# HBioquant/DiffBindFR

Measured on AMD Instinct MI355X. Metric: poses_per_sec, higher is better.
Workload: dtype f32

## Files before the change

### diffbindfr_amd/csrc/api.cpp

```cpp
#include <cmath>
#include <cstdio>
#include <cstring>
#include <algorithm>
#include <atomic>
#include <map>

#include "common.h"

void launch_conv(const ConvArgs& a, hipStream_t st);
void launch_conv_layer(const ConvArgs* c4, hipStream_t st);
void launch_conv2(const Conv2Args& a, hipStream_t st);
void launch_conv2h(const Conv2Args& a, hipStream_t st);
void launch_convz(const ConvZArgs& a, hipStream_t st);
void launch_reduce_ln(const float* msg, const int* row_start, const int* row_cnt, int N, int D, const LNDesc& ln,
                      const float* old, int D_old, float* out, int ldo, int mode, hipStream_t st, const uint8_t* first = nullptr, unsigned long long sc_lanes = 0);
struct ReduceLayerArgs {
  const float* msg[4]; const int* row_start[4]; const int* row_cnt[4]; LNDesc ln[4];
  int NL, NA, D, D_old;
  const float* old_l; const float* old_a; float* out_l; float* out_a;
  const uint8_t* first[4]; unsigned long long sc_lanes[4];
};
static unsigned long long convz_sc_lanes(const ConvZ& z) {
  unsigned long long m = 0;
  for (int i = 0; i < z.n_io; ++i) m |= 0xfffull << (z.out_off[i] / 4);
// ... 7 lines not shown
  float lig_cut2, atom_cut2, cross_cut2;
  int lig_cap, atom_cap, dynamic_cross;
  EdgeSet set[N_SETS];
  int* err;
  int step, lds_nl, lds_na, n_chunk, lanes;
};
void dbfr_edge_form(const dbfr_batch& b, int* n_chunk, int* lanes);
void launch_edges(const GraphArgs& A, bool heads_only, hipStream_t st);
void launch_edge_log(const GraphArgs& A, int* log_row, int stride, hipStream_t st);
void launch_edge_ties(const GraphArgs& A, int* log_row, int stride, float tol, hipStream_t st);
void launch_graph_chunks(const GraphArgs& A, hipStream_t st);
void launch_flat_chunks(const int* tgt, const int* n_edges, int max_edges, int span, int n_span, int* cnt0, int cap, int* chunk_es, int* chunk_gl, hipStream_t st);
void launch_row_absmax(const float* lx, const int* lig_ptr, float* out_l, const float* ax, const int* atm_ptr, float* out_a, int ld, int D, int G, int n_rows_a, hipStream_t st);
void launch_batch_vectors(const dbfr_batch& b, int* lig_batch, int* atm_batch, uint8_t* is_cab, int* n_cab,
                          int* tor_batch, int* sc_batch, hipStream_t st);
void launch_time_embed(const float* t, int G, float emb_scale, float* temb, hipStream_t st);
enum MlpIn { IN_LIGNODE = 0, IN_LIGEDGE = 1, IN_TG = 2, IN_G = 3 };
struct MlpArgs {
  Mlp2 w; int mode; const int* n_rows_dev; int n_rows_max; const float* temb; const int* row_graph_tab; const int* tgt;
  const int* aux; const float* dist; const float* bond_feat; int nfeat; const float* lig_node; int nnode;
  const float* gs_offset; const float* gs_coeff; float* out;
};
void launch_mlp(const MlpArgs& a, hipStream_t st);
struct AtomEncArgs {
  const float* pocket_feat; const int* atm_batch; const float* temb; const float* emb[5]; int dims[5];
  const float* lin_t; int NA; float* out;
};
void launch_atom_encoder(const AtomEncArgs& a, hipStream_t st);
void launch_center_edges(const dbfr_batch& b, int* tgt, int* gth, float* dist, float* sh, int* row_start, int* row_cnt,
                         hipStream_t st);
struct TrRotArgs {
  const float* gp; const float* temb; const float* tr_sigma; const float* rot_norm; Mlp2 tr, rot; int G;
  int scale_by_sigma; float* tr_out; float* rot_out; int* err;
};
void launch_trrot(const TrRotArgs& a, hipStream_t st);
void launch_bond_attr(const float* x, int ldx, const int* b0, const int* b1, const int* bsel, int stride, int n,
                      float* out, hipStream_t st);
void launch_tor_final(const float* feat, const Mlp2& w, const float* norm2, int scale, int n, float* out, hipStream_t st);
struct SdeLigArgs {
  dbfr_batch b; const float* tr_score; const float* rot_score; const float* tor_score; const float* z_tr;
  const float* z_rot; const float* z_tor; float dt, tr_g2, tr_gsdt, rot_g2, rot_gsdt, tor_g2, tor_gsdt; float* traj;
  int* err;
};
void launch_sde_ligand(const SdeLigArgs& a, hipStream_t st);
void launch_sidechain(const dbfr_batch& b, const float* score, const float* z, float dt, float g2, float gsdt,
                      const int* a14_group, float* atom14_out, float* traj14, const int* err, hipStream_t st);
// ... 1072 lines not shown
  ga.lig_cut2 = cfg.lig_cutoff * cfg.lig_cutoff; ga.atom_cut2 = cfg.atom_cutoff * cfg.atom_cutoff;
  ga.cross_cut2 = cfg.dynamic_max_cross ? 1.0f : cfg.cross_cutoff * cfg.cross_cutoff;
  ga.lig_cap = cfg.lig_max_neighbors; ga.atom_cap = cfg.atom_max_neighbors; ga.dynamic_cross = cfg.dynamic_max_cross;
  for (int k = 0; k < N_SETS; ++k) ga.set[k] = w.set[k];
  ga.err = w.err; ga.step = step; ga.lds_nl = ga.lds_na = 0;
  dbfr_edge_form(*B, &ga.n_chunk, &ga.lanes);
  launch_edges(ga, false, st);
  if (int lrc = take_launch_error()) return lrc;
  if (m->gemm_split == DBFR_GEMM_REDUCE_FIRST) launch_graph_chunks(ga, st);
  if (m->edge_log && step < m->edge_log_steps) launch_edge_log(ga, m->edge_log + (size_t)step * N_SETS * m->edge_log_graphs, m->edge_log_graphs, st);
  if (m->tie_log && step < m->tie_log_steps) launch_edge_ties(ga, m->tie_log + (size_t)step * N_SETS * m->tie_log_graphs, m->tie_log_graphs, m->tie_tol, st);
  {
    MlpArgs a; memset(&a, 0, sizeof a);
    a.w = m->lig_node_emb; a.mode = IN_LIGNODE; a.n_rows_max = NL; a.temb = w.temb; a.row_graph_tab = w.lig_batch;
    a.lig_node = B->lig_node; a.nnode = cfg.lig_node_features; a.out = w.lig_x[0];
    launch_mlp(a, st);
  }
  {
    AtomEncArgs a; a.pocket_feat = B->pocket_feat; a.atm_batch = w.atm_batch; a.temb = w.temb;
    for (int i = 0; i < 5; ++i) { a.emb[i] = m->atom_emb[i]; a.dims[i] = m->atom_dims[i]; }
    a.lin_t = m->atom_lin_t; a.NA = NA; a.out = w.atom_x[0];
    launch_atom_encoder(a, st);
  }
  auto edge_mlp = [&](const Mlp2& mw, int mode, const EdgeSet& S, const int* tab, const float* off, const float* co) {
    MlpArgs a; memset(&a, 0, sizeof a);
    a.w = mw; a.mode = mode; a.n_rows_dev = S.n_edges; a.n_rows_max = S.cap; a.temb = w.temb; a.row_graph_tab = tab;
    a.tgt = S.tgt; a.aux = S.aux; a.dist = S.dist; a.bond_feat = B->bond_feat; a.nfeat = cfg.lig_edge_features;
    a.gs_offset = off; a.gs_coeff = co; a.out = S.emb;
    launch_mlp(a, st);
  };
  edge_mlp(m->lig_edge_emb, IN_LIGEDGE, w.set[SET_LL], w.lig_batch, m->gs_lig_off, m->gs_lig_c);
  edge_mlp(m->atom_edge_emb, IN_TG, w.set[SET_AA], w.atm_batch, m->gs_atom_off, m->gs_atom_c);
  edge_mlp(m->la_edge_emb, IN_TG, w.set[SET_AL], w.lig_batch, m->gs_cross_off, m->gs_cross_c);
  edge_mlp(m->la_edge_emb, IN_TG, w.set[SET_LA], w.atm_batch, m->gs_cross_off, m->gs_cross_c);
  static const int dims[4] = {48, 84, 120, 168};
  int cur = 0;
  for (int l = 0; l < cfg.num_conv_layers; ++l) {
    const int Di = dims[std::min(l, 3)], Do = dims[std::min(l + 1, 3)];
    const float *lx = w.lig_x[cur], *ax = w.atom_x[cur];
    float *lnew = w.lig_x[cur ^ 1], *anew = w.atom_x[cur ^ 1];
    const EdgeSet &LL = w.set[SET_LL], &AA = w.set[SET_AA], &AL = w.set[SET_AL], &LA = w.set[SET_LA];
    if (w.conv2 || l < m->conv2_layers) {
      const bool rf = m->gemm_split == DBFR_GEMM_REDUCE_FIRST && !((m->layer_fallback >> l) & 1u);
      const ConvW2* L2 = rf ? m->layer2v[l] : m->layer2[l];
      const Conv2Desc ds[4] = {
          conv2_desc(L2[0], LL.n_edges, LL.cap, LL.gth, LL.emb, LL.sh, lx, Di, LL.tgt, lx, Di, LL.gth, lx, Di, w.msg[0]),
          conv2_desc(L2[1], AL.n_edges, AL.cap, AL.gth, AL.emb, AL.sh, lx, Di, AL.tgt, ax, Di, AL.gth, ax, Di, w.msg[1]),
          conv2_desc(L2[2], AA.n_edges, AA.cap, AA.gth, AA.emb, AA.sh, ax, Di, AA.tgt, ax, Di, AA.gth, ax, Di, w.msg[2]),
          conv2_desc(L2[3], LA.n_edges, LA.cap, LA.gth, LA.emb, LA.sh, ax, Di, LA.tgt, lx, Di, LA.gth, lx, Di, w.msg[3])};
      const int Ws[4] = {m->layer[l][0].W, m->layer[l][1].W, m->layer[l][2].W, m->layer[l][3].W};
      if (rf) {
        launch_row_absmax(lx, B->lig_ptr, w.xmax_l, ax, B->atm_ptr, w.xmax_a, Di, Di, G, NA, st);
      }
      auto zd = [&](int i, const EdgeSet& S, const float* xmax) { return convz_desc(ds[i], m->layerz[l][i], S.tgt, Do, S.chunk_es, S.chunk_gl, S.chunk0 + G, S.chunk_cap, xmax); };
      const ConvZDesc zs[4] = {zd(0, LL, w.xmax_l), zd(1, AL, w.xmax_a), zd(2, AA, w.xmax_a), zd(3, LA, w.xmax_l)};
      conv2_call(m, ds, Ws, 4, st, (m->layer_fallback >> l) & 1u, rf ? zs : nullptr);
      ReduceLayerArgs ra;
// ... 481 lines not shown
extern "C" int dbfr_test_conv2(dbfr_model* m, int32_t layer, int32_t family, int32_t n_edges, const int32_t* n_edges_dev,
                               const int32_t* tgt, const int32_t* gth, const float* emb, const float* sh,
                               const float* tab1, int32_t ld1, const int32_t* idx1, const float* tab2, int32_t ld2,
                               const int32_t* idx2, const float* x, int32_t ldx, float* msg, void* hip_stream) {
  return test_conv_impl(m, true, layer, family, n_edges, n_edges_dev, tgt, gth, emb, sh, tab1, ld1, idx1, tab2, ld2, idx2, x, ldx,
                        msg, hip_stream);
}

extern "C" int dbfr_test_reduce_ln2(dbfr_model* m, int32_t layer, int32_t family, const float* msg, const int32_t* row_start, const int32_t* row_cnt,
                                    int32_t n_nodes, const float* old, int32_t d_old, float* out, int32_t mode, const uint8_t* seg_first, void* hip_stream) {
  if (!m) return fail(DBFR_ERR_ARG, "null model");
  const ConvW* cw = pick_conv(m, layer, family);
  if (!cw) return fail(DBFR_ERR_ARG, "no such conv");
  unsigned long long lanes = 0;
  if (seg_first) {
    if (layer == -1 || cw->K != 144) return fail(DBFR_ERR_ARG, "dbfr_test_reduce_ln2: seg_first with a conv that has no reduce-first form");
    lanes = convz_sc_lanes(layer >= 0 ? m->layerz[layer][family] : layer == -2 ? m->tor_convz : m->sc_convz);
  }
  launch_reduce_ln(msg, row_start, row_cnt, n_nodes, cw->D_out, cw->ln, old, d_old, out, cw->D_out, mode, (hipStream_t)hip_stream, seg_first, lanes);
  HIPCHECK(hipGetLastError());
  return DBFR_OK;
}

extern "C" int dbfr_test_reduce_ln(dbfr_model* m, int32_t layer, int32_t family, const float* msg,
                                   const int32_t* row_start, const int32_t* row_cnt, int32_t n_nodes, const float* old,
                                   int32_t d_old, float* out, int32_t mode, void* hip_stream) {
  if (!m) return fail(DBFR_ERR_ARG, "null model");
  const ConvW* cw = pick_conv(m, layer, family);
  if (!cw) return fail(DBFR_ERR_ARG, "no such conv");
  launch_reduce_ln(msg, row_start, row_cnt, n_nodes, cw->D_out, cw->ln, old, d_old, out, cw->D_out, mode,
                   (hipStream_t)hip_stream);
  HIPCHECK(hipGetLastError());
  return DBFR_OK;
}
```

### diffbindfr_amd/csrc/conv.hip

```cpp
#include <cstdio>
#include <cstdlib>
#include <type_traits>
#include <vector>

#include "common.h"

#ifndef CONV_PRIO
#define CONV_PRIO 0
#endif
#ifndef CONV_XPF
#define CONV_XPF 0
#endif
#ifndef CONV_NB2_WAVES
#define CONV_NB2_WAVES 2
#endif
#define XS_LD (MAXD + 4)

typedef float f32x4 __attribute__((ext_vector_type(4)));

#define TRACE_BLOCKS 1024
#define TRACE_TILES 48
#define TRACE_REC (2 + 3 * TRACE_TILES + 8)
#define RSTAMP(k) do { if ((ABL & 16) && a.trace && bid < TRACE_BLOCKS && lane == 0) a.trace[((size_t)bid * 4 + wave) * TRACE_REC + 2 + 3 * TRACE_TILES + (k)] = __builtin_amdgcn_s_memrealtime(); } while (0)
#define TSTAMP(k) do { if ((ABL & 16) && a.trace && bid < TRACE_BLOCKS && lane == 0) a.trace[((size_t)bid * 4 + wave) * TRACE_REC + 2 + 3 * TRACE_TILES + (k)] = __builtin_readcyclecounter(); } while (0)
// ... 500 lines not shown
      float v = buf[wave][c];
      float* o = out + (size_t)node * ldo + c;
      if (mode == 0) v = (c < D_old ? old[(size_t)node * D_old + c] : 0.f) + v;
      else if (mode == 1) v = *o + v;
      *o = v;
    }
  }
}

void launch_reduce_ln(const float* msg, const int* row_start, const int* row_cnt, int N, int D, const LNDesc& ln,
                      const float* old, int D_old, float* out, int ldo, int mode, hipStream_t st, const uint8_t* first, unsigned long long sc_lanes) {
  if (N <= 0) return;
  hipLaunchKernelGGL(k_reduce_ln, dim3((N + 3) / 4), dim3(256), 0, st, msg, row_start, row_cnt, N, D, ln, old, D_old,
                     out, ldo, mode, first, sc_lanes);
}

struct ReduceLayerArgs {
  const float* msg[4]; const int* row_start[4]; const int* row_cnt[4]; LNDesc ln[4];
  int NL, NA, D, D_old;
  const float* old_l; const float* old_a; float* out_l; float* out_a;
  const uint8_t* first[4]; unsigned long long sc_lanes[4];
};

__device__ __forceinline__ void mean_ln(const float* __restrict__ msg, int rs, int rc, int D, const LNDesc& ln, float* bw, int lane, const uint8_t* first, unsigned long long sc_lanes) {
  const int d4 = D >> 2;
  const f32x4 acc = row_sum(msg, rs, rc, D, lane, first, sc_lanes);
  if (lane < d4) {
    const float cntf = (float)max(rc, 1);
    bw[4 * lane] = acc[0] / cntf; bw[4 * lane + 1] = acc[1] / cntf; bw[4 * lane + 2] = acc[2] / cntf; bw[4 * lane + 3] = acc[3] / cntf;
  }
  __builtin_amdgcn_wave_barrier();
  int iw = 0, ib = 0;
  for (int bk = 0; bk < ln.nblk; ++bk) {
    const int mul = ln.mul[bk], dim = ln.dim[bk], off = ln.off[bk];
    const int nel = mul * dim;
    float mean[3] = {0.f, 0.f, 0.f};
    const bool d3 = dim == 3;
    for (int i = lane; i < nel; i += 64) {
      int comp = d3 ? i % 3 : 0;
      float v = bw[off + i];
      if (comp == 0) mean[0] += v; else if (comp == 1) mean[1] += v; else mean[2] += v;
    }
    for (int o = 32; o > 0; o >>= 1) mean[0] += __shfl_xor(mean[0], o);
    mean[0] /= (float)mul;
    if (d3) {
#pragma unroll
      for (int c = 1; c < 3; ++c) {
        for (int o = 32; o > 0; o >>= 1) mean[c] += __shfl_xor(mean[c], o);
        mean[c] /= (float)mul;
      }
    }
    float sq = 0.f;
    for (int i = lane; i < nel; i += 64) {
      int u = d3 ? i / 3 : i, comp = d3 ? i - 3 * u : 0;
      float v = bw[off + i] - (comp == 0 ? mean[0] : comp == 1 ? mean[1] : mean[2]) * ln.mean_shift[iw + u];
      bw[off + i] = v;
      sq += v * v;
    }
    __builtin_amdgcn_wave_barrier();
    for (int o = 32; o > 0; o >>= 1) sq += __shfl_xor(sq, o);
    const float inv = 1.0f / sqrtf(sq / (float)nel + 1e-5f);
    for (int i = lane; i < nel; i += 64) {
      int u = d3 ? i / 3 : i;
      float v = bw[off + i] * (inv * ln.weight[iw + u]);
      if (ln.is0e[bk]) v += ln.bias[ib + u];
      bw[off + i] = v;
    }
    iw += mul;
    if (ln.is0e[bk]) ib += mul;
  }
  __builtin_amdgcn_wave_barrier();
}

__global__ __launch_bounds__(256) void k_reduce_ln_layer(ReduceLayerArgs a) {
  __shared__ float buf[4][2][MAXD];
  const int lane = threadIdx.x & 63, wave = threadIdx.x >> 6;
  const int nbl = (a.NL + 3) / 4;
  const bool lig = (int)blockIdx.x < nbl;
  const int node = (lig ? blockIdx.x : blockIdx.x - nbl) * 4 + wave;
  const int N = lig ? a.NL : a.NA;
  if (node >= N) return;
  const int s0 = lig ? 0 : 2;
  mean_ln(a.msg[s0], a.row_start[s0][node], a.row_cnt[s0][node], a.D, a.ln[s0], buf[wave][0], lane, a.first[s0], a.sc_lanes[s0]);
  mean_ln(a.msg[s0 + 1], a.row_start[s0 + 1][node], a.row_cnt[s0 + 1][node], a.D, a.ln[s0 + 1], buf[wave][1], lane, a.first[s0 + 1], a.sc_lanes[s0 + 1]);
  const float* old = (lig ? a.old_l : a.old_a) + (size_t)node * a.D_old;
  float* out = (lig ? a.out_l : a.out_a) + (size_t)node * a.D;
#pragma unroll
  for (int j = 0; j < 3; ++j) {
    const int c = lane + 64 * j;
    if (c < a.D) out[c] = ((c < a.D_old ? old[c] : 0.f) + buf[wave][0][c]) + buf[wave][1][c];
  }
}

void launch_reduce_ln_layer(const ReduceLayerArgs& a, hipStream_t st) {
  const int nb = (a.NL + 3) / 4 + (a.NA + 3) / 4;
  if (nb <= 0) return;
  hipLaunchKernelGGL(k_reduce_ln_layer, dim3(nb), dim3(256), 0, st, a);
}
```

### diffbindfr_amd/csrc/graph.hip

```cpp
#include "common.h"

#define MAX_NL 256
#define MAX_NA 8192

enum SetKind { SET_LL = 0, SET_AA = 1, SET_AL = 2, SET_LA = 3, SET_TOR = 4, SET_SC = 5, N_SETS = 6 };

struct GraphArgs {
  dbfr_batch b;
  const int* lig_batch;
  const int* atm_batch;
  const uint8_t* is_cab;
  const int* n_cab;
  const float* tr_sigma;
  float lig_cut2, atom_cut2, cross_cut2;
  int lig_cap, atom_cap, dynamic_cross;
  EdgeSet set[N_SETS];
  int* err;
  int step;
  int lds_nl, lds_na;
  int n_chunk;
  int lanes;
};

__device__ __forceinline__ float d2_rn(float ax, float ay, float az, float bx, float by, float bz) {
// ... 747 lines not shown
#pragma unroll
  for (int t = 0; t < 3; ++t)
#pragma unroll
    for (int r = 0; r < 4; ++r) acc[t][r] = a.w.b1 ? a.w.b1[16 * t + 4 * g + r] : 0.f;
#pragma unroll
  for (int k = 0; k < NS; k += 4) {
    const float bv = hid[row][k + g];
#pragma unroll
    for (int t = 0; t < 3; ++t) acc[t] = __builtin_amdgcn_mfma_f32_16x16x4f32(w1[(k + g) * NS + 16 * t + n], bv, acc[t], 0, 0, 0);
  }
  if (row < nr) {
#pragma unroll
    for (int t = 0; t < 3; ++t) *reinterpret_cast<f32x4*>(a.out + (size_t)(r0 + row) * NS + 16 * t + 4 * g) = acc[t];
  }
  }
}

void launch_mlp(const MlpArgs& a, hipStream_t st) {
  if (a.n_rows_max <= 0) return;
  const int tiles = (a.n_rows_max + MLP_ROWS - 1) / MLP_ROWS;
  hipLaunchKernelGGL(k_mlp, dim3(tiles < 1024 ? tiles : 1024), dim3(256), 0, st, a);
}

struct AtomEncArgs {
  const float* pocket_feat;
  const int* atm_batch;
  const float* temb;
  const float* emb[5];
  int dims[5];
  const float* lin_t;
  int NA;
  float* out;
};

__global__ __launch_bounds__(256) void k_atom_encoder(AtomEncArgs a) {
  __shared__ float w[(NS + EMB) * NS];
  __shared__ float x[16][NS + EMB];
  for (int i = threadIdx.x; i < (NS + EMB) * NS; i += 256) w[i] = a.lin_t[i];
  const int r0 = blockIdx.x * 16;
  for (int i = threadIdx.x; i < 16 * (NS + EMB); i += 256) {
    int r = i / (NS + EMB), c = i % (NS + EMB);
    int row = r0 + r;
    float v = 0.f;
    if (row < a.NA) {
      if (c < NS) {
        for (int f = 0; f < 5; ++f) {
// ... 26 lines not shown
```

### diffbindfr_amd/lib.py

```python
import ctypes as C
import os

HERE = os.path.dirname(os.path.abspath(__file__))
LIB_PATH = os.environ.get("DBFR_LIB") or os.path.join(HERE, "libdbfr.so")

DBFR_OK = 0
DBFR_ERR_CAPACITY = -3
ERRORS = {-1: "DBFR_ERR_ARG", -2: "DBFR_ERR_HIP", -3: "DBFR_ERR_CAPACITY", -4: "DBFR_ERR_SELFTEST",
          -5: "DBFR_ERR_NUMERIC"}

i32, f32, vp = C.c_int32, C.c_float, C.c_void_p


class ModelCfg(C.Structure):
    _fields_ = [(n, i32) for n in ("ns", "nv", "sh_lmax", "num_conv_layers", "lig_node_features",
                                   "lig_edge_features", "distance_embed_dim", "sigma_embed_dim")] + \
               [(n, f32) for n in ("emb_scale", "lig_cutoff", "atom_cutoff", "cross_cutoff", "center_max_distance")] + \
               [(n, i32) for n in ("atom_max_neighbors", "lig_max_neighbors", "dynamic_max_cross", "scale_by_sigma",
                                   "no_sc_torsion")]


class Tensor(C.Structure):
    _fields_ = [("name", C.c_char_p), ("data", vp), ("numel", C.c_int64)]

# ... 132 lines not shown
               [(n, vp) for n in ("lig", "pos14", "center", "static_pos", "map_ptr", "atom_map", "file_map", "frame_file",
                                  "frame_src", "frame_step")]


class XtcOpts(C.Structure):
    _fields_ = [("precision", f32), ("dt", f32), ("first_step", i32), ("box", f32 * 9)]


class SitesOpts(C.Structure):
    _fields_ = [(n, f32) for n in ("spacing", "probe", "ray_length", "lining_cutoff")] + \
               [(n, i32) for n in ("min_buried", "min_points", "max_sites")]


class SitesIn(C.Structure):
    _fields_ = [("n_prot", i32), ("n_res", i32), ("max_points", C.c_int64)] + \
               [(n, vp) for n in ("res_ptr", "aatype", "atom37_pos", "atom37_mask", "radius")]


class SitesOut(C.Structure):
    _fields_ = [(n, vp) for n in ("n_sites", "label", "n_points", "score", "idx_sum", "centre", "lining", "grid", "occupancy",
                                  "burial", "labels")]


SYMBOLS = ["dbfr_model_create", "dbfr_model_destroy", "dbfr_model_set_edge_log", "dbfr_model_set_tie_log", "dbfr_model_fallback_convs", "dbfr_model_rowscaled_convs", "dbfr_model_set_gemm", "dbfr_model_get_gemm", "dbfr_workspace_bytes", "dbfr_score", "dbfr_sample",
           "dbfr_sample_range", "dbfr_capacity_report",
           "dbfr_init_poses", "dbfr_extract_templates", "dbfr_status_sync", "dbfr_abi_version", "dbfr_build_id", "dbfr_last_error", "dbfr_wigner3j", "dbfr_conv_paths", "dbfr_test_pack_f16_tiles", "dbfr_test_pack_f16_rows", "dbfr_test_chunk_table", "dbfr_test_pack_f16_depth", "dbfr_probe_mfma_f16",
           "dbfr_profile_enable", "dbfr_profile_read", "dbfr_profile_fused_bytes", "dbfr_profile_executed_flops", "dbfr_profile_useful_flops", "dbfr_workspace_layout", "dbfr_test_conv", "dbfr_test_conv2", "dbfr_test_reduce_ln", "dbfr_test_reduce_ln2", "dbfr_test_sde_step",
           "dbfr_pose_metrics", "dbfr_pdb_format", "dbfr_pdb_write_files", "dbfr_select_pocket", "dbfr_sdf_format",
           "dbfr_sdf_write_files", "dbfr_mdn_model_create", "dbfr_mdn_model_destroy", "dbfr_mdn_workspace_bytes", "dbfr_mdn_forward", "dbfr_mdn_pocket_features",
           "dbfr_vina_workspace_bytes", "dbfr_vina_score", "dbfr_vina_score_at", "dbfr_vina_minimize",
           "dbfr_pose_rmsd_matrix", "dbfr_select_modes", "dbfr_pose_check",
           "dbfr_pdb_atom_map", "dbfr_complex_pdb_format", "dbfr_complex_pdb_write_files", "dbfr_xtc_workspace_bytes", "dbfr_xtc_encode",
           "dbfr_sites_workspace_bytes", "dbfr_find_sites", "dbfr_interactions"]

_lib = None


class DbfrError(RuntimeError):
    pass


def load():
    global _lib
    if _lib is not None:
        return _lib
    if not os.path.exists(LIB_PATH):
        raise DbfrError(f"{LIB_PATH} is missing: build the HIP library first "
                        f"(python -m diffbindfr_amd.build). There is no CPU fallback.")
    lib = C.CDLL(LIB_PATH)
    lib.dbfr_last_error.restype = C.c_char_p
# ... 17 lines not shown
    lib.dbfr_capacity_report.argtypes = [vp, vp, C.POINTER(i32), C.POINTER(C.c_int64)]
    lib.dbfr_init_poses.argtypes = [vp, C.POINTER(Batch), C.POINTER(InitTape), vp, vp]
    lib.dbfr_extract_templates.argtypes = [i32, vp, vp, vp, vp, vp, vp, vp, vp]
    lib.dbfr_status_sync.argtypes = [vp, vp, C.POINTER(C.c_int64)]
    lib.dbfr_wigner3j.argtypes = [i32, i32, i32, C.POINTER(C.c_double)]
    lib.dbfr_conv_paths.argtypes = [i32, C.POINTER(i32), i32, C.POINTER(i32)]
    lib.dbfr_test_pack_f16_tiles.argtypes = [vp, vp, i32, vp, C.POINTER(i32)]
    lib.dbfr_test_pack_f16_depth.argtypes = [vp, vp, i32, C.POINTER(i32), C.POINTER(i32)]
    lib.dbfr_test_pack_f16_rows.argtypes = [vp, vp, i32, vp, C.POINTER(i32), vp, C.POINTER(i32)]
    lib.dbfr_test_chunk_table.argtypes = [vp, vp, i32, i32, vp, i32, vp, vp, vp]
    lib.dbfr_probe_mfma_f16.argtypes = [C.c_double, C.POINTER(C.c_double), vp]
    lib.dbfr_profile_enable.argtypes = [vp, i32]
    lib.dbfr_profile_fused_bytes.argtypes = [vp, C.POINTER(C.c_double)]
    lib.dbfr_profile_executed_flops.argtypes = [vp, C.POINTER(C.c_double)]
    lib.dbfr_profile_useful_flops.argtypes = [vp, C.POINTER(C.c_double), C.POINTER(C.c_double)]
    lib.dbfr_profile_read.argtypes = [vp, C.POINTER(C.c_double), C.POINTER(C.c_int64), C.POINTER(C.c_double),
                                      C.POINTER(C.c_double), i32]
    lib.dbfr_workspace_layout.argtypes = [vp, C.POINTER(Batch), C.POINTER(Limits), C.c_char_p, C.c_size_t,
                                          C.POINTER(C.c_size_t), C.POINTER(C.c_size_t), i32]
    lib.dbfr_test_conv.argtypes = [vp, i32, i32, i32, vp, vp, vp, vp, vp, vp, i32, vp, vp, i32, vp, vp, i32, vp, vp]
    lib.dbfr_test_conv2.argtypes = lib.dbfr_test_conv.argtypes
    lib.dbfr_test_reduce_ln.argtypes = [vp, i32, i32, vp, vp, vp, i32, vp, i32, vp, i32, vp]
    lib.dbfr_test_reduce_ln2.argtypes = [vp, i32, i32, vp, vp, vp, i32, vp, i32, vp, i32, vp, vp]
    lib.dbfr_test_sde_step.argtypes = [vp, C.POINTER(Batch), C.POINTER(Step), C.POINTER(Scores), C.POINTER(Noise), vp, vp, vp]
    lib.dbfr_select_pocket.argtypes = [i32, i32, vp, i32, vp, vp, vp, vp, C.c_double, i32, vp, vp, vp]
    lib.dbfr_pose_metrics.argtypes = [C.POINTER(PoseMetricsIn), C.POINTER(PoseMetricsOut), vp]
    lib.dbfr_pdb_format.argtypes = [C.POINTER(PdbTopology), i32, vp, vp, i32, i32, vp, C.c_int64]
    lib.dbfr_pdb_format.restype = C.c_int64
    lib.dbfr_pdb_write_files.argtypes = [C.POINTER(PdbTopology), i32, vp, vp, i32, C.POINTER(C.c_char_p), i32]
    lib.dbfr_sdf_format.argtypes = [C.POINTER(SdfTemplate), vp, vp, C.c_int64]
    lib.dbfr_sdf_format.restype = C.c_int64
    lib.dbfr_sdf_write_files.argtypes = [C.POINTER(SdfTemplate), vp, i32, C.POINTER(C.c_char_p), i32]
    lib.dbfr_mdn_model_create.argtypes = [C.POINTER(Tensor), i32, C.POINTER(vp)]
    lib.dbfr_mdn_model_destroy.argtypes = [vp]
    lib.dbfr_mdn_model_destroy.restype = None
    lib.dbfr_mdn_workspace_bytes.argtypes = [C.POINTER(MdnBatch), C.POINTER(C.c_size_t)]
    lib.dbfr_mdn_pocket_features.argtypes = [i32, i32, vp, vp, vp, vp, i32, vp, vp, vp, vp, vp, vp, vp, vp]
    lib.dbfr_mdn_forward.argtypes = [vp, C.POINTER(MdnBatch), vp, vp, vp, vp, C.c_size_t, vp]
    lib.dbfr_vina_workspace_bytes.argtypes = [C.POINTER(VinaIn), C.POINTER(C.c_size_t)]
    lib.dbfr_vina_score.argtypes = [C.POINTER(VinaIn), vp, vp, vp, vp, C.c_size_t, vp]
    lib.dbfr_vina_score_at.argtypes = [C.POINTER(VinaIn), vp, vp, vp, vp, vp, vp, vp, C.c_size_t, vp]
    lib.dbfr_vina_minimize.argtypes = [C.POINTER(VinaIn), C.POINTER(VinaOpts), vp, vp, vp, vp, C.c_size_t, vp]
    lib.dbfr_pose_rmsd_matrix.argtypes = [C.POINTER(PoseRmsdIn), vp, vp]
    lib.dbfr_select_modes.argtypes = [C.POINTER(PoseRmsdIn), vp, vp, C.POINTER(ModesOpts), vp, vp, vp, vp]
    lib.dbfr_pose_check.argtypes = [C.POINTER(PoseCheckIn), C.POINTER(PoseCheckOpts), C.POINTER(PoseCheckOut), vp]
    lib.dbfr_pdb_atom_map.argtypes = [C.POINTER(PdbTopology), i32, vp, vp, vp, C.c_int64, C.POINTER(C.c_int64)]
# ... 35 lines not shown
```

### include/dbfr.h

```cpp
#ifndef DBFR_H
#define DBFR_H

#include <stddef.h>
#include <stdint.h>

#ifdef __cplusplus
extern "C" {
#endif

#define DBFR_ABI_VERSION 7

typedef enum {
  DBFR_OK = 0,
  DBFR_ERR_ARG = -1,
  DBFR_ERR_HIP = -2,
  DBFR_ERR_CAPACITY = -3,
  DBFR_ERR_SELFTEST = -4,
  DBFR_ERR_NUMERIC = -5
} dbfr_status;

typedef struct dbfr_model dbfr_model;

typedef struct {
  int32_t ns, nv, sh_lmax;
// ... 496 lines not shown
int dbfr_profile_fused_bytes(const dbfr_model* m, double* fused_form_bytes);
int dbfr_profile_executed_flops(const dbfr_model* m, double* executed_flops);
int dbfr_profile_useful_flops(const dbfr_model* m, double* useful_flops, double* form_bytes);

int dbfr_probe_mfma_f16(double seconds, double* tflops, void* hip_stream);

int dbfr_workspace_layout(const dbfr_model* m, const dbfr_batch* b, const dbfr_limits* lim, char* names,
                          size_t names_cap, size_t* offsets, size_t* bytes, int32_t max_entries);

int dbfr_test_conv(dbfr_model* m, int32_t layer, int32_t family, int32_t n_edges, const int32_t* n_edges_dev,
                   const int32_t* tgt, const int32_t* gth, const float* emb, const float* sh, const float* tab1,
                   int32_t ld1, const int32_t* idx1, const float* tab2, int32_t ld2, const int32_t* idx2,
                   const float* x, int32_t ldx, float* msg, void* hip_stream);
int dbfr_test_conv2(dbfr_model* m, int32_t layer, int32_t family, int32_t n_edges, const int32_t* n_edges_dev,
                    const int32_t* tgt, const int32_t* gth, const float* emb, const float* sh, const float* tab1,
                    int32_t ld1, const int32_t* idx1, const float* tab2, int32_t ld2, const int32_t* idx2,
                    const float* x, int32_t ldx, float* msg, void* hip_stream);
int dbfr_test_reduce_ln(dbfr_model* m, int32_t layer, int32_t family, const float* msg, const int32_t* row_start,
                        const int32_t* row_cnt, int32_t n_nodes, const float* old, int32_t d_old, float* out,
                        int32_t mode, void* hip_stream);
int dbfr_test_reduce_ln2(dbfr_model* m, int32_t layer, int32_t family, const float* msg, const int32_t* row_start,
                         const int32_t* row_cnt, int32_t n_nodes, const float* old, int32_t d_old, float* out,
                         int32_t mode, const uint8_t* seg_first, void* hip_stream);

int dbfr_test_sde_step(const dbfr_model* m, const dbfr_batch* b, const dbfr_step* step, const dbfr_scores* scores,
                       const dbfr_noise* z, float* atom14_out, int32_t* err_word_out, void* hip_stream);

#ifdef __cplusplus
}
#endif
#endif
```

Measured before the change: 480.4.

## Fuse four edge-embedding MLPs into one MFMA kernel; persist reduce-LN layer kernel

Result: no change. 482.6 (median of 3 runs) (+0.5%).

```diff
diff --git a/diffbindfr_amd/csrc/api.cpp b/diffbindfr_amd/csrc/api.cpp
--- a/diffbindfr_amd/csrc/api.cpp
+++ b/diffbindfr_amd/csrc/api.cpp
@@ -53,6 +53,12 @@
   const float* gs_offset; const float* gs_coeff; float* out;
 };
 void launch_mlp(const MlpArgs& a, hipStream_t st);
+struct EdgeMlpSet {
+  Mlp2 w; int mode; const int* n_rows_dev; int n_rows_max; const int* row_graph_tab; const int* tgt; const int* aux; const float* dist;
+  const float* gs_offset; const float* gs_coeff; float* out;
+};
+struct EdgeMlpArgs { EdgeMlpSet set[4]; int n_sets; const float* temb; const float* bond_feat; int nfeat; };
+void launch_edge_mlp(const EdgeMlpArgs& a, bool via_k_mlp, hipStream_t st);
 struct AtomEncArgs {
   const float* pocket_feat; const int* atm_batch; const float* temb; const float* emb[5]; int dims[5];
   const float* lin_t; int NA; float* out;
@@ -1171,17 +1177,20 @@
     a.lin_t = m->atom_lin_t; a.NA = NA; a.out = w.atom_x[0];
     launch_atom_encoder(a, st);
   }
-  auto edge_mlp = [&](const Mlp2& mw, int mode, const EdgeSet& S, const int* tab, const float* off, const float* co) {
-    MlpArgs a; memset(&a, 0, sizeof a);
-    a.w = mw; a.mode = mode; a.n_rows_dev = S.n_edges; a.n_rows_max = S.cap; a.temb = w.temb; a.row_graph_tab = tab;
-    a.tgt = S.tgt; a.aux = S.aux; a.dist = S.dist; a.bond_feat = B->bond_feat; a.nfeat = cfg.lig_edge_features;
-    a.gs_offset = off; a.gs_coeff = co; a.out = S.emb;
-    launch_mlp(a, st);
-  };
-  edge_mlp(m->lig_edge_emb, IN_LIGEDGE, w.set[SET_LL], w.lig_batch, m->gs_lig_off, m->gs_lig_c);
-  edge_mlp(m->atom_edge_emb, IN_TG, w.set[SET_AA], w.atm_batch, m->gs_atom_off, m->gs_atom_c);
-  edge_mlp(m->la_edge_emb, IN_TG, w.set[SET_AL], w.lig_batch, m->gs_cross_off, m->gs_cross_c);
-  edge_mlp(m->la_edge_emb, IN_TG, w.set[SET_LA], w.atm_batch, m->gs_cross_off, m->gs_cross_c);
+  {
+    EdgeMlpArgs ea; memset(&ea, 0, sizeof ea);
+    auto edge_set = [&](const Mlp2& mw, int mode, const EdgeSet& S, const int* tab, const float* off, const float* co) {
+      EdgeMlpSet& e = ea.set[ea.n_sets++];
+      e.w = mw; e.mode = mode; e.n_rows_dev = S.n_edges; e.n_rows_max = S.cap; e.row_graph_tab = tab; e.tgt = S.tgt; e.aux = S.aux; e.dist = S.dist;
+      e.gs_offset = off; e.gs_coeff = co; e.out = S.emb;
+    };
+    edge_set(m->lig_edge_emb, IN_LIGEDGE, w.set[SET_LL], w.lig_batch, m->gs_lig_off, m->gs_lig_c);
+    edge_set(m->atom_edge_emb, IN_TG, w.set[SET_AA], w.atm_batch, m->gs_atom_off, m->gs_atom_c);
+    edge_set(m->la_edge_emb, IN_TG, w.set[SET_AL], w.lig_batch, m->gs_cross_off, m->gs_cross_c);
+    edge_set(m->la_edge_emb, IN_TG, w.set[SET_LA], w.atm_batch, m->gs_cross_off, m->gs_cross_c);
+    ea.temb = w.temb; ea.bond_feat = B->bond_feat; ea.nfeat = cfg.lig_edge_features;
+    launch_edge_mlp(ea, false, st);
+  }
   static const int dims[4] = {48, 84, 120, 168};
   int cur = 0;
   for (int l = 0; l < cfg.num_conv_layers; ++l) {
@@ -1709,6 +1718,49 @@
   return DBFR_OK;
 }
 
+extern "C" int dbfr_test_reduce_ln_layer(dbfr_model* m, int32_t layer, const float* const* msg, const int32_t* const* row_start,
+                                         const int32_t* const* row_cnt, const uint8_t* const* seg_first, int32_t n_lig, int32_t n_atom,
+                                         const float* old_l, const float* old_a, int32_t d_old, float* out_l, float* out_a, void* hip_stream) {
+  if (!m) return fail(DBFR_ERR_ARG, "null model");
+  if (layer < 0 || layer >= m->cfg.num_conv_layers || !msg || !row_start || !row_cnt || n_lig < 0 || n_atom < 0)
+    return fail(DBFR_ERR_ARG, "dbfr_test_reduce_ln_layer: bad argument");
+  ReduceLayerArgs ra;
+  for (int i = 0; i < 4; ++i) {
+    const ConvW* cw = pick_conv(m, layer, i);
+    if (!cw) return fail(DBFR_ERR_ARG, "no such conv");
+    if (seg_first && cw->K != 144) return fail(DBFR_ERR_ARG, "dbfr_test_reduce_ln_layer: seg_first with a conv that has no reduce-first form");
+    ra.msg[i] = msg[i]; ra.row_start[i] = row_start[i]; ra.row_cnt[i] = row_cnt[i]; ra.ln[i] = cw->ln;
+    ra.first[i] = seg_first ? seg_first[i] : nullptr;
+    ra.sc_lanes[i] = seg_first ? convz_sc_lanes(m->layerz[layer][i]) : 0;
+    ra.D = cw->D_out;
+  }
+  ra.NL = n_lig; ra.NA = n_atom; ra.D_old = d_old; ra.old_l = old_l; ra.old_a = old_a; ra.out_l = out_l; ra.out_a = out_a;
+  launch_reduce_ln_layer(ra, (hipStream_t)hip_stream);
+  HIPCHECK(hipGetLastError());
+  return DBFR_OK;
+}
+
+extern "C" int dbfr_test_edge_mlp(dbfr_model* m, int32_t n_sets, const dbfr_test_edge_set* sets, const float* temb, const float* bond_feat,
+                                  int32_t via_k_mlp, void* hip_stream) {
+  if (!m) return fail(DBFR_ERR_ARG, "null model");
+  if (n_sets < 1 || n_sets > 4 || !sets || !temb) return fail(DBFR_ERR_ARG, "dbfr_test_edge_mlp: bad argument");
+  EdgeMlpArgs ea; memset(&ea, 0, sizeof ea);
+  for (int i = 0; i < n_sets; ++i) {
+    const dbfr_test_edge_set& s = sets[i];
+    if (s.kind < 0 || s.kind > 3 || s.n_rows_max < 0 || (s.kind == 0 && !bond_feat)) return fail(DBFR_ERR_ARG, "dbfr_test_edge_mlp: bad edge set");
+    EdgeMlpSet& e = ea.set[i];
+    e.w = s.kind == 0 ? m->lig_edge_emb : s.kind == 1 ? m->atom_edge_emb : m->la_edge_emb;
+    e.mode = s.kind == 0 ? IN_LIGEDGE : IN_TG;
+    e.gs_offset = s.kind == 0 ? m->gs_lig_off : s.kind == 1 ? m->gs_atom_off : m->gs_cross_off;
+    e.gs_coeff = s.kind == 0 ? m->gs_lig_c : s.kind == 1 ? m->gs_atom_c : m->gs_cross_c;
+    e.n_rows_dev = s.n_rows_dev; e.n_rows_max = s.n_rows_max; e.row_graph_tab = s.batch_tab; e.tgt = s.tgt; e.aux = s.aux; e.dist = s.dist; e.out = s.out;
+  }
+  ea.n_sets = n_sets; ea.temb = temb; ea.bond_feat = bond_feat; ea.nfeat = m->cfg.lig_edge_features;
+  launch_edge_mlp(ea, via_k_mlp != 0, (hipStream_t)hip_stream);
+  HIPCHECK(hipGetLastError());
+  return DBFR_OK;
+}
+
 extern "C" int dbfr_test_reduce_ln(dbfr_model* m, int32_t layer, int32_t family, const float* msg,
                                    const int32_t* row_start, const int32_t* row_cnt, int32_t n_nodes, const float* old,
                                    int32_t d_old, float* out, int32_t mode, void* hip_stream) {
diff --git a/diffbindfr_amd/csrc/conv.hip b/diffbindfr_amd/csrc/conv.hip
--- a/diffbindfr_amd/csrc/conv.hip
+++ b/diffbindfr_amd/csrc/conv.hip
@@ -546,24 +546,25 @@
   const uint8_t* first[4]; unsigned long long sc_lanes[4];
 };
 
-__device__ __forceinline__ void mean_ln(const float* __restrict__ msg, int rs, int rc, int D, const LNDesc& ln, float* bw, int lane, const uint8_t* first, unsigned long long sc_lanes) {
-  const int d4 = D >> 2;
-  const f32x4 acc = row_sum(msg, rs, rc, D, lane, first, sc_lanes);
-  if (lane < d4) {
-    const float cntf = (float)max(rc, 1);
-    bw[4 * lane] = acc[0] / cntf; bw[4 * lane + 1] = acc[1] / cntf; bw[4 * lane + 2] = acc[2] / cntf; bw[4 * lane + 3] = acc[3] / cntf;
-  }
-  __builtin_amdgcn_wave_barrier();
-  int iw = 0, ib = 0;
+__device__ __forceinline__ void ln_row(float* bw, const LNDesc& ln, const float* __restrict__ par, int lane) {
+#pragma clang fp contract(off)
+  static_assert(MAXD <= 192, "three elements per lane cover an irreps block");
+  const float *p_shift = par, *p_weight = par + MAXD, *p_bias = par + 2 * MAXD;
   for (int bk = 0; bk < ln.nblk; ++bk) {
-    const int mul = ln.mul[bk], dim = ln.dim[bk], off = ln.off[bk];
-    const int nel = mul * dim;
-    float mean[3] = {0.f, 0.f, 0.f};
-    const bool d3 = dim == 3;
-    for (int i = lane; i < nel; i += 64) {
-      int comp = d3 ? i % 3 : 0;
-      float v = bw[off + i];
-      if (comp == 0) mean[0] += v; else if (comp == 1) mean[1] += v; else mean[2] += v;
+    const int mul = ln.mul[bk], off = ln.off[bk];
+    const bool d3 = ln.dim[bk] == 3, b0e = ln.is0e[bk] != 0;
+    const int nel = d3 ? 3 * mul : mul;
+    float v[3] = {0.f, 0.f, 0.f}, mean[3] = {0.f, 0.f, 0.f};
+#pragma unroll
+    for (int j = 0; j < 3; ++j) {
+      if (64 * j < nel) {
+        const int i = lane + 64 * j;
+        if (i < nel) {
+          const int comp = d3 ? i % 3 : 0;
+          v[j] = bw[off + i];
+          if (comp == 0) mean[0] += v[j]; else if (comp == 1) mean[1] += v[j]; else mean[2] += v[j];
+        }
+      }
     }
     for (int o = 32; o > 0; o >>= 1) mean[0] += __shfl_xor(mean[0], o);
     mean[0] /= (float)mul;
@@ -575,49 +576,96 @@
       }
     }
     float sq = 0.f;
-    for (int i = lane; i < nel; i += 64) {
-      int u = d3 ? i / 3 : i, comp = d3 ? i - 3 * u : 0;
-      float v = bw[off + i] - (comp == 0 ? mean[0] : comp == 1 ? mean[1] : mean[2]) * ln.mean_shift[iw + u];
-      bw[off + i] = v;
-      sq += v * v;
-    }
-    __builtin_amdgcn_wave_barrier();
+#pragma unroll
+    for (int j = 0; j < 3; ++j) {
+      if (64 * j < nel) {
+        const int i = lane + 64 * j;
+        if (i < nel) {
+          const int comp = d3 ? i % 3 : 0;
+          v[j] = __builtin_fmaf(-(comp == 0 ? mean[0] : comp == 1 ? mean[1] : mean[2]), p_shift[off + i], v[j]);
+          sq = __builtin_fmaf(v[j], v[j], sq);
+        }
+      }
+    }
     for (int o = 32; o > 0; o >>= 1) sq += __shfl_xor(sq, o);
     const float inv = 1.0f / sqrtf(sq / (float)nel + 1e-5f);
-    for (int i = lane; i < nel; i += 64) {
-      int u = d3 ? i / 3 : i;
-      float v = bw[off + i] * (inv * ln.weight[iw + u]);
-      if (ln.is0e[bk]) v += ln.bias[ib + u];
-      bw[off + i] = v;
-    }
-    iw += mul;
-    if (ln.is0e[bk]) ib += mul;
-  }
-  __builtin_amdgcn_wave_barrier();
+#pragma unroll
+    for (int j = 0; j < 3; ++j) {
+      if (64 * j < nel) {
+        const int i = lane + 64 * j;
+        if (i < nel) {
+          float r = v[j] * (inv * p_weight[off + i]);
+          if (b0e) r += p_bias[off + i];
+          bw[off + i] = r;
+        }
+      }
+    }
+  }
 }
 
 __global__ __launch_bounds__(256) void k_reduce_ln_layer(ReduceLayerArgs a) {
-  __shared__ float buf[4][2][MAXD];
-  const int lane = threadIdx.x & 63, wave = threadIdx.x >> 6;
-  const int nbl = (a.NL + 3) / 4;
-  const bool lig = (int)blockIdx.x < nbl;
-  const int node = (lig ? blockIdx.x : blockIdx.x - nbl) * 4 + wave;
-  const int N = lig ? a.NL : a.NA;
-  if (node >= N) return;
-  const int s0 = lig ? 0 : 2;
-  mean_ln(a.msg[s0], a.row_start[s0][node], a.row_cnt[s0][node], a.D, a.ln[s0], buf[wave][0], lane, a.first[s0], a.sc_lanes[s0]);
-  mean_ln(a.msg[s0 + 1], a.row_start[s0 + 1][node], a.row_cnt[s0 + 1][node], a.D, a.ln[s0 + 1], buf[wave][1], lane, a.first[s0 + 1], a.sc_lanes[s0 + 1]);
-  const float* old = (lig ? a.old_l : a.old_a) + (size_t)node * a.D_old;
-  float* out = (lig ? a.out_l : a.out_a) + (size_t)node * a.D;
-#pragma unroll
-  for (int j = 0; j < 3; ++j) {
-    const int c = lane + 64 * j;
-    if (c < a.D) out[c] = ((c < a.D_old ? old[c] : 0.f) + buf[wave][0][c]) + buf[wave][1][c];
+  __shared__ __attribute__((aligned(16))) float buf[4][2][MAXD];
+  __shared__ float par[4][3][MAXD];
+  const int lane = threadIdx.x & 63, wave = __builtin_amdgcn_readfirstlane(threadIdx.x >> 6);
+  const int D = a.D, d4 = D >> 2;
+#pragma unroll
+  for (int s = 0; s < 4; ++s) {
+    const LNDesc& ln = a.ln[s];
+    const int e = threadIdx.x;
+    if (e < D) {
+      float sh = 0.f, wg = 0.f, bi = 0.f;
+      int iw = 0, ib = 0;
+      for (int bk = 0; bk < ln.nblk; ++bk) {
+        const int mul = ln.mul[bk], dim = ln.dim[bk], i = e - ln.off[bk];
+        if (i >= 0 && i < mul * dim) {
+          const int u = dim == 3 ? i / 3 : i;
+          sh = ln.mean_shift[iw + u]; wg = ln.weight[iw + u];
+          if (ln.is0e[bk]) bi = ln.bias[ib + u];
+        }
+        iw += mul;
+        if (ln.is0e[bk]) ib += mul;
+      }
+      par[s][0][e] = sh; par[s][1][e] = wg; par[s][2][e] = bi;
+    }
+  }
+  __syncthreads();
+  const int ntot = a.NL + a.NA;
+  float* b0 = buf[wave][0];
+  float* b1 = buf[wave][1];
+  for (int n = blockIdx.x * 4 + wave; n < ntot; n += gridDim.x * 4) {
+    const bool lig = n < a.NL;
+    const int node = lig ? n : n - a.NL, s0 = lig ? 0 : 2;
+    const int rs0 = a.row_start[s0][node], rc0 = a.row_cnt[s0][node], rs1 = a.row_start[s0 + 1][node], rc1 = a.row_cnt[s0 + 1][node];
+    const float* old = (lig ? a.old_l : a.old_a) + (size_t)node * a.D_old;
+    float* out = (lig ? a.out_l : a.out_a) + (size_t)node * D;
+    const f32x4 acc0 = row_sum(a.msg[s0], rs0, rc0, D, lane, a.first[s0], a.sc_lanes[s0]);
+    const f32x4 acc1 = row_sum(a.msg[s0 + 1], rs1, rc1, D, lane, a.first[s0 + 1], a.sc_lanes[s0 + 1]);
+    if (lane < d4) {
+      const float c0 = (float)max(rc0, 1), c1 = (float)max(rc1, 1);
+      f32x4 m0, m1;
+#pragma unroll
+      for (int r = 0; r < 4; ++r) { m0[r] = acc0[r] / c0; m1[r] = acc1[r] / c1; }
+      *reinterpret_cast<f32x4*>(b0 + 4 * lane) = m0;
+      *reinterpret_cast<f32x4*>(b1 + 4 * lane) = m1;
+    }
+    __builtin_amdgcn_wave_barrier();
+    ln_row(b0, a.ln[s0], par[s0][0], lane);
+    ln_row(b1, a.ln[s0 + 1], par[s0 + 1][0], lane);
+    __builtin_amdgcn_wave_barrier();
+#pragma unroll
+    for (int j = 0; j < 3; ++j) {
+      const int c = lane + 64 * j;
+      if (c < D) out[c] = ((c < a.D_old ? old[c] : 0.f) + b0[c]) + b1[c];
+    }
+    __builtin_amdgcn_wave_barrier();
   }
 }
 
 void launch_reduce_ln_layer(const ReduceLayerArgs& a, hipStream_t st) {
-  const int nb = (a.NL + 3) / 4 + (a.NA + 3) / 4;
+  const int nb = (a.NL + a.NA + 3) / 4;
   if (nb <= 0) return;
-  hipLaunchKernelGGL(k_reduce_ln_layer, dim3(nb), dim3(256), 0, st, a);
-}
+  static int per_cu = 0;
+  if (per_cu <= 0 && (hipOccupancyMaxActiveBlocksPerMultiprocessor(&per_cu, k_reduce_ln_layer, 256, 0) != hipSuccess || per_cu <= 0)) per_cu = 4;
+  const int cap = per_cu * dbfr_current_cu_count();
+  hipLaunchKernelGGL(k_reduce_ln_layer, dim3(nb < cap ? nb : cap), dim3(256), 0, st, a);
+}
diff --git a/diffbindfr_amd/csrc/graph.hip b/diffbindfr_amd/csrc/graph.hip
--- a/diffbindfr_amd/csrc/graph.hip
+++ b/diffbindfr_amd/csrc/graph.hip
@@ -793,6 +793,149 @@
   hipLaunchKernelGGL(k_mlp, dim3(tiles < 1024 ? tiles : 1024), dim3(256), 0, st, a);
 }
 
+struct EdgeMlpSet {
+  Mlp2 w; int mode; const int* n_rows_dev; int n_rows_max; const int* row_graph_tab; const int* tgt; const int* aux; const float* dist;
+  const float* gs_offset; const float* gs_coeff; float* out;
+};
+struct EdgeMlpArgs { EdgeMlpSet set[4]; int n_sets; const float* temb; const float* bond_feat; int nfeat; };
+
+#define EMLP_LD (MLP_MAXIN + 1)
+
+template <int NK>
+__device__ __forceinline__ void edge_mlp_units(const EdgeMlpArgs& a, const EdgeMlpSet& S, int nrows, int u0, int u1, float (*xw)[EMLP_LD], const float* s_gs) {
+  typedef float f32x4 __attribute__((ext_vector_type(4)));
+  const int lane = threadIdx.x & 63, wave = threadIdx.x >> 6, n = lane & 15, g = lane >> 4;
+  const int in = S.w.in;
+  float w0r[NK][3], w1r[NS / 4][3];
+#pragma unroll
+  for (int ks = 0; ks < NK; ++ks)
+#pragma unroll
+    for (int t = 0; t < 3; ++t) w0r[ks][t] = 4 * ks + g < in ? S.w.w0t[(4 * ks + g) * NS + 16 * t + n] : 0.f;
+#pragma unroll
+  for (int ks = 0; ks < NS / 4; ++ks)
+#pragma unroll
+    for (int t = 0; t < 3; ++t) w1r[ks][t] = S.w.w1t[(4 * ks + g) * NS + 16 * t + n];
+  const float coeff = S.gs_coeff ? S.gs_coeff[0] : 0.f;
+  const int rl = lane >> 2, q = lane & 3;
+  for (int u = u0; u < u1; ++u) {
+    const int r0 = u * MLP_ROWS;
+    const int nr = min(MLP_ROWS, nrows - r0);
+    {
+      const int r = 16 * wave + rl;
+      const bool live = r < nr;
+      const int arow = r0 + (live ? r : 0);
+      const int gph = S.row_graph_tab[S.tgt ? S.tgt[arow] : arow];
+      const float dcl = fminf(S.dist[arow], s_gs[EMB - 1]);
+      const int bond = S.mode == IN_LIGEDGE ? S.aux[arow] : -1;
+      for (int c = q; c < in; c += 4) {
+        float v = 0.f;
+        if (live) {
+          int cc = c;
+          if (S.mode == IN_LIGEDGE) {
+            if (cc < a.nfeat) { v = bond >= 0 ? a.bond_feat[(size_t)bond * a.nfeat + cc] : 0.f; cc = -1; }
+            else cc -= a.nfeat;
+          }
+          if (cc >= 0) {
+            if (cc < EMB) v = a.temb[gph * EMB + cc];
+            else {
+              const float d = dcl - s_gs[cc - EMB];
+              v = expf(coeff * (d * d));
+            }
+          }
+        }
+        xw[rl][c] = v;
+      }
+      if (4 * NK > in)
+        for (int i = lane; i < 16 * (4 * NK - in); i += 64) xw[i / (4 * NK - in)][in + i % (4 * NK - in)] = 0.f;
+    }
+    __builtin_amdgcn_wave_barrier();
+    f32x4 acc[3];
+#pragma unroll
+    for (int t = 0; t < 3; ++t)
+#pragma unroll
+      for (int r = 0; r < 4; ++r) acc[t][r] = S.w.b0 ? S.w.b0[16 * t + 4 * g + r] : 0.f;
+#pragma unroll
+    for (int ks = 0; ks < NK; ++ks) {
+      const float bv = xw[n][4 * ks + g];
+#pragma unroll
+      for (int t = 0; t < 3; ++t) acc[t] = __builtin_amdgcn_mfma_f32_16x16x4f32(w0r[ks][t], bv, acc[t], 0, 0, 0);
+    }
+    __builtin_amdgcn_wave_barrier();
+#pragma unroll
+    for (int t = 0; t < 3; ++t)
+#pragma unroll
+      for (int r = 0; r < 4; ++r) xw[n][16 * t + 4 * g + r] = fmaxf(acc[t][r], 0.f);
+    __builtin_amdgcn_wave_barrier();
+#pragma unroll
+    for (int t = 0; t < 3; ++t)
+#pragma unroll
+      for (int r = 0; r < 4; ++r) acc[t][r] = S.w.b1 ? S.w.b1[16 * t + 4 * g + r] : 0.f;
+#pragma unroll
+    for (int ks = 0; ks < NS / 4; ++ks) {
+      const float bv = xw[n][4 * ks + g];
+#pragma unroll
+      for (int t = 0; t < 3; ++t) acc[t] = __builtin_amdgcn_mfma_f32_16x16x4f32(w1r[ks][t], bv, acc[t], 0, 0, 0);
+    }
+    const int row = 16 * wave + n;
+    if (row < nr) {
+#pragma unroll
+      for (int t = 0; t < 3; ++t) *reinterpret_cast<f32x4*>(S.out + (size_t)(r0 + row) * NS + 16 * t + 4 * g) = acc[t];
+    }
+    __builtin_amdgcn_wave_barrier();
+  }
+}
+
+__global__ __launch_bounds__(256, 3) void k_edge_mlp(EdgeMlpArgs a) {
+  __shared__ float xw[4][16][EMLP_LD];
+  __shared__ float s_gs[EMB];
+  const int wave = threadIdx.x >> 6;
+  auto rows_of = [&](int s) { return max(a.set[s].n_rows_dev ? min(*a.set[s].n_rows_dev, a.set[s].n_rows_max) : a.set[s].n_rows_max, 0); };
+  int total = 0;
+  for (int s = 0; s < a.n_sets; ++s) total += (rows_of(s) + MLP_ROWS - 1) / MLP_ROWS;
+  const int lo = (int)((long)blockIdx.x * total / gridDim.x), hi = (int)((long)(blockIdx.x + 1) * total / gridDim.x);
+  int base = 0;
+#pragma unroll 1
+  for (int s = 0; s < a.n_sets; ++s) {
+    const int nrows = rows_of(s), tiles = (nrows + MLP_ROWS - 1) / MLP_ROWS;
+    const int u0 = max(lo, base) - base, u1 = min(hi, base + tiles) - base;
+    base += tiles;
+    if (u0 >= u1) continue;
+    const EdgeMlpSet& S = a.set[s];
+    __syncthreads();
+    if (threadIdx.x < EMB) s_gs[threadIdx.x] = S.gs_offset ? S.gs_offset[threadIdx.x] : 0.f;
+    __syncthreads();
+    if (((S.w.in + 3) & ~3) == 76) edge_mlp_units<19>(a, S, nrows, u0, u1, xw[wave], s_gs);
+    else edge_mlp_units<16>(a, S, nrows, u0, u1, xw[wave], s_gs);
+  }
+}
+
+void launch_edge_mlp(const EdgeMlpArgs& a, bool via_k_mlp, hipStream_t st) {
+  long tiles = 0;
+  bool fits = true;
+  for (int i = 0; i < a.n_sets; ++i) {
+    const EdgeMlpSet& s = a.set[i];
+    const int kin = (s.w.in + 3) & ~3;
+    fits = fits && (kin == 64 || kin == 76) && s.w.in > EMB && (s.mode == IN_TG || (s.mode == IN_LIGEDGE && s.w.in == a.nfeat + 2 * EMB)) && (s.mode != IN_TG || s.w.in == 2 * EMB) && s.dist && s.row_graph_tab;
+    tiles += (std::max(s.n_rows_max, 0) + MLP_ROWS - 1) / MLP_ROWS;
+  }
+  if (!via_k_mlp && fits) {
+    if (tiles <= 0) return;
+    static int per_cu = 0;
+    if (per_cu <= 0 && (hipOccupancyMaxActiveBlocksPerMultiprocessor(&per_cu, k_edge_mlp, 256, 0) != hipSuccess || per_cu <= 0)) per_cu = 2;
+    const long cap = (long)per_cu * dbfr_current_cu_count();
+    hipLaunchKernelGGL(k_edge_mlp, dim3((unsigned)std::min(tiles, cap)), dim3(256), 0, st, a);
+    return;
+  }
+  for (int i = 0; i < a.n_sets; ++i) {
+    const EdgeMlpSet& s = a.set[i];
+    MlpArgs m; memset(&m, 0, sizeof m);
+    m.w = s.w; m.mode = s.mode; m.n_rows_dev = s.n_rows_dev; m.n_rows_max = s.n_rows_max; m.temb = a.temb; m.row_graph_tab = s.row_graph_tab;
+    m.tgt = s.tgt; m.aux = s.aux; m.dist = s.dist; m.bond_feat = a.bond_feat; m.nfeat = a.nfeat; m.gs_offset = s.gs_offset; m.gs_coeff = s.gs_coeff;
+    m.out = s.out;
+    launch_mlp(m, st);
+  }
+}
+
 struct AtomEncArgs {
   const float* pocket_feat;
   const int* atm_batch;
diff --git a/diffbindfr_amd/lib.py b/diffbindfr_amd/lib.py
--- a/diffbindfr_amd/lib.py
+++ b/diffbindfr_amd/lib.py
@@ -178,10 +178,14 @@
                                   "burial", "labels")]
 
 
+class TestEdgeSet(C.Structure):
+    _fields_ = [("kind", i32), ("n_rows_max", i32)] + [(n, vp) for n in ("n_rows_dev", "tgt", "aux", "dist", "batch_tab", "out")]
+
+
 SYMBOLS = ["dbfr_model_create", "dbfr_model_destroy", "dbfr_model_set_edge_log", "dbfr_model_set_tie_log", "dbfr_model_fallback_convs", "dbfr_model_rowscaled_convs", "dbfr_model_set_gemm", "dbfr_model_get_gemm", "dbfr_workspace_bytes", "dbfr_score", "dbfr_sample",
            "dbfr_sample_range", "dbfr_capacity_report",
            "dbfr_init_poses", "dbfr_extract_templates", "dbfr_status_sync", "dbfr_abi_version", "dbfr_build_id", "dbfr_last_error", "dbfr_wigner3j", "dbfr_conv_paths", "dbfr_test_pack_f16_tiles", "dbfr_test_pack_f16_rows", "dbfr_test_chunk_table", "dbfr_test_pack_f16_depth", "dbfr_probe_mfma_f16",
-           "dbfr_profile_enable", "dbfr_profile_read", "dbfr_profile_fused_bytes", "dbfr_profile_executed_flops", "dbfr_profile_useful_flops", "dbfr_workspace_layout", "dbfr_test_conv", "dbfr_test_conv2", "dbfr_test_reduce_ln", "dbfr_test_reduce_ln2", "dbfr_test_sde_step",
+           "dbfr_profile_enable", "dbfr_profile_read", "dbfr_profile_fused_bytes", "dbfr_profile_executed_flops", "dbfr_profile_useful_flops", "dbfr_workspace_layout", "dbfr_test_conv", "dbfr_test_conv2", "dbfr_test_reduce_ln", "dbfr_test_reduce_ln2", "dbfr_test_reduce_ln_layer", "dbfr_test_edge_mlp", "dbfr_test_sde_step",
            "dbfr_pose_metrics", "dbfr_pdb_format", "dbfr_pdb_write_files", "dbfr_select_pocket", "dbfr_sdf_format",
            "dbfr_sdf_write_files", "dbfr_mdn_model_create", "dbfr_mdn_model_destroy", "dbfr_mdn_workspace_bytes", "dbfr_mdn_forward", "dbfr_mdn_pocket_features",
            "dbfr_vina_workspace_bytes", "dbfr_vina_score", "dbfr_vina_score_at", "dbfr_vina_minimize",
@@ -245,6 +249,8 @@
     lib.dbfr_test_conv2.argtypes = lib.dbfr_test_conv.argtypes
     lib.dbfr_test_reduce_ln.argtypes = [vp, i32, i32, vp, vp, vp, i32, vp, i32, vp, i32, vp]
     lib.dbfr_test_reduce_ln2.argtypes = [vp, i32, i32, vp, vp, vp, i32, vp, i32, vp, i32, vp, vp]
+    lib.dbfr_test_reduce_ln_layer.argtypes = [vp, i32, C.POINTER(vp), C.POINTER(vp), C.POINTER(vp), C.POINTER(vp), i32, i32, vp, vp, i32, vp, vp, vp]
+    lib.dbfr_test_edge_mlp.argtypes = [vp, i32, C.POINTER(TestEdgeSet), vp, vp, i32, vp]
     lib.dbfr_test_sde_step.argtypes = [vp, C.POINTER(Batch), C.POINTER(Step), C.POINTER(Scores), C.POINTER(Noise), vp, vp, vp]
     lib.dbfr_select_pocket.argtypes = [i32, i32, vp, i32, vp, vp, vp, vp, C.c_double, i32, vp, vp, vp]
     lib.dbfr_pose_metrics.argtypes = [C.POINTER(PoseMetricsIn), C.POINTER(PoseMetricsOut), vp]
diff --git a/include/dbfr.h b/include/dbfr.h
--- a/include/dbfr.h
+++ b/include/dbfr.h
@@ -542,6 +542,21 @@
 int dbfr_test_reduce_ln2(dbfr_model* m, int32_t layer, int32_t family, const float* msg, const int32_t* row_start,
                          const int32_t* row_cnt, int32_t n_nodes, const float* old, int32_t d_old, float* out,
                          int32_t mode, const uint8_t* seg_first, void* hip_stream);
+int dbfr_test_reduce_ln_layer(dbfr_model* m, int32_t layer, const float* const* msg, const int32_t* const* row_start,
+                              const int32_t* const* row_cnt, const uint8_t* const* seg_first, int32_t n_lig, int32_t n_atom,
+                              const float* old_l, const float* old_a, int32_t d_old, float* out_l, float* out_a, void* hip_stream);
+
+typedef struct dbfr_test_edge_set {
+  int32_t kind, n_rows_max;
+  const int32_t* n_rows_dev;
+  const int32_t* tgt;
+  const int32_t* aux;
+  const float* dist;
+  const int32_t* batch_tab;
+  float* out;
+} dbfr_test_edge_set;
+int dbfr_test_edge_mlp(dbfr_model* m, int32_t n_sets, const dbfr_test_edge_set* sets, const float* temb, const float* bond_feat,
+                       int32_t via_k_mlp, void* hip_stream);
 
 int dbfr_test_sde_step(const dbfr_model* m, const dbfr_batch* b, const dbfr_step* step, const dbfr_scores* scores,
                        const dbfr_noise* z, float* atom14_out, int32_t* err_word_out, void* hip_stream);
```
